# voithru/voice-activity-detection

Hardware: AMD Instinct MI355X
Metric: audio frames/sec (whole node) (higher is better)
Workload: dtype f32 (bf16x6 split operands, f32 accumulate)

## Files before the change

### voice_activity_detection_amd/csrc/savad.hip

```cpp
#include "savad_kernels.h"
#include "savad_kernels_bf16.h"
#include "savad_attn_pw_bf16.h"
#include "savad_packed_bf16.h"
#include "savad_kernels_f32s.h"
#include "savad_generic.h"
#include <type_traits>
#include "savad_logmel.h"
#include "savad_frontend.h"
#include "savad_ingest.h"
#include "savad_post.h"
#include "savad_post_device.h"
#include "savad_schedule.h"

#include <math.h>
#include <stdarg.h>
#include <stdio.h>
#include <string.h>

#include <functional>
#include <map>
#include <mutex>
#include <string>
#include <vector>

// ... 40 lines not shown
    size_t raw_floats = 0, packed_floats = 0;
    bool dirty = true;
    float* d_pe = nullptr;
    int pe_len = 0;
    std::vector<float> h_pe;
    int splits = 0;
    int row_mode = 0;
    bool batch_invariant = false;
    int precision = 0;
    char* d_frag3 = nullptr;
    size_t frag3_bytes = 0;
    bool frag3_dirty = true;
    bool lds_attrs3_set = false;
    size_t f3_win = 0;
    unsigned* d_sat = nullptr;
    char* d_frag = nullptr;
    size_t frag_bytes = 0;
    bool frag_dirty = true;
    bool lds_attrs_set = false;
    int n_cu = 256;
    size_t f_win = 0;
    struct LayerFrag {
        size_t wqkv, wo, w1, w2;
        size_t wqkv_vo = 0;
    };
    std::vector<LayerFrag> lf;
    std::vector<LayerFrag> lf3;
    int prof_capacity = 0, prof_used = 0, prof_nk = 0, prof_skip = 0;
    std::vector<hipEvent_t> events;
    std::vector<const char*> knames;

    size_t r_win, r_bin, r_lnf_w, r_lnf_b, r_wc, r_bc;
    struct LayerRaw {
        size_t wq, bq, wk, bk, wv, bv, wo, bo, ln1w, ln1b, w1, b1, w2, b2, ln2w, ln2b;
    };
    std::vector<LayerRaw> lr;
    struct LayerPacked {
        size_t wqkv, bqkv, w1, b1;
        size_t wvo, bqkv_vo;
        size_t frag;
    };
    std::vector<LayerPacked> lp;
    size_t p_wc, p_bc;
    size_t p_bias = 0;
    int FP = 0;
    size_t p_win_pad = 0;
};

namespace {

using namespace savad;

size_t add_param(savad_model* m, const std::string& key, size_t numel) {
    const size_t off = m->raw_floats;
    m->params.push_back(Param{key, numel, off, false});
    m->raw_floats += (numel + 3) & ~size_t(3);
    return off;
}

static_assert(sched::D == D && sched::TILE == TILE && sched::F32_MAX_LAYERS == PACKED_MAX_LAYERS, "savad_schedule.h: savad_kernels.h sizes");
static_assert(sched::BF_BLK_BYTES == bf::BLK_BYTES && sched::BF_HBLK_FLOATS == bf::HBLK_FLOATS && sched::BF_HRES_BYTES == sizeof(bf::hres_t) &&
                  sched::BF16_MAX_LAYERS == bf::PACKED_BF16_MAX_LAYERS && sched::PW_GRID == bf::PW_GRID, "savad_schedule.h: bf16 sizes");
// ... 129 lines not shown
    m->frag_dirty = false;
    return SAVAD_OK;
}

int pack_frags3(savad_model* m, hipStream_t st, const float* W, int N, int K, size_t off) {
    const size_t total = (size_t)N * K;
    const int grid = (int)((total + 255) / 256 < 1024 ? (total + 255) / 256 : 1024);
    hipLaunchKernelGGL(fs::pack_weight_frags3_kernel, dim3(grid), dim3(256), 0, st, W, N, K, reinterpret_cast<__bf16*>(m->d_frag3 + off));
    HIP_TRY(hipGetLastError());
    return SAVAD_OK;
}

int prepare_frags3(savad_model* m, hipStream_t st) {
    if (!m->frag3_dirty) return SAVAD_OK;
    const int L = m->cfg.num_layers;
    int rc;
    if ((rc = pack_frags3(m, st, win_fp32(m), D, m->FP, m->f3_win))) return rc;
    for (int l = 0; l < L; ++l) {
        if ((rc = pack_frags3(m, st, m->d_packed + m->lp[l].wqkv, 3 * D, D, m->lf3[l].wqkv))) return rc;
        if ((rc = pack_frags3(m, st, m->d_raw + m->lr[l].wo, D, D, m->lf3[l].wo))) return rc;
        if ((rc = pack_frags3(m, st, m->d_packed + m->lp[l].w1, DFF, D, m->lf3[l].w1))) return rc;
        if ((rc = pack_frags3(m, st, m->d_raw + m->lr[l].w2, D, DFF, m->lf3[l].w2))) return rc;
        const auto& p = m->lp[l];
        hipLaunchKernelGGL(fs::fold_vo_kernel, dim3(D), dim3(D), 0, st, m->d_raw + m->lr[l].wo, m->d_packed + p.wqkv + (size_t)2 * D * D,
                           m->d_packed + p.bqkv, m->d_packed + p.wvo, m->d_packed + p.bqkv_vo);
        HIP_TRY(hipGetLastError());
        if ((rc = pack_frags3(m, st, m->d_packed + p.wqkv, 2 * D, D, m->lf3[l].wqkv_vo))) return rc;
        if ((rc = pack_frags3(m, st, m->d_packed + p.wvo, D, D, m->lf3[l].wqkv_vo + (size_t)2 * D * D * 6))) return rc;
    }
    m->frag3_dirty = false;
    return SAVAD_OK;
}

template <typename KernelT>
int allow_lds(KernelT kernel, int bytes) {
    HIP_TRY(hipFuncSetAttribute(reinterpret_cast<const void*>(kernel), hipFuncAttributeMaxDynamicSharedMemorySize, bytes));
    return SAVAD_OK;
}

struct Prof {
    savad_model* m;
    hipStream_t st;
    hipEvent_t* ev;
    int n;
    Prof(savad_model* mm, hipStream_t s) : m(mm), st(s), ev(nullptr), n(0) {
        if (m->prof_capacity > 0 && m->prof_skip > 0) {
            --m->prof_skip;
        } else if (m->prof_capacity > 0 && m->prof_used < m->prof_capacity) {
            ev = m->events.data() + (size_t)m->prof_used * MAX_EVENTS;
            m->knames.clear();
            hipEventRecord(ev[0], st);
// ... 195 lines not shown
        r.wk = add_param(m, p + "self_attention.key_projection.weight", (size_t)D * D);
        r.bk = add_param(m, p + "self_attention.key_projection.bias", D);
        r.wv = add_param(m, p + "self_attention.value_projection.weight", (size_t)D * D);
        r.bv = add_param(m, p + "self_attention.value_projection.bias", D);
        r.wo = add_param(m, p + "self_attention.final_projection.weight", (size_t)D * D);
        r.bo = add_param(m, p + "self_attention.final_projection.bias", D);
        r.ln1w = add_param(m, p + "self_attention_sublayer.layer_norm.weight", D);
        r.ln1b = add_param(m, p + "self_attention_sublayer.layer_norm.bias", D);
        r.w1 = add_param(m, p + "feed_forward.feed_forward.0.weight", (size_t)DFF * D);
        r.b1 = add_param(m, p + "feed_forward.feed_forward.0.bias", DFF);
        r.w2 = add_param(m, p + "feed_forward.feed_forward.3.weight", (size_t)D * DFF);
        r.b2 = add_param(m, p + "feed_forward.feed_forward.3.bias", D);
        r.ln2w = add_param(m, p + "feed_forward_sublayer.layer_norm.weight", D);
        r.ln2b = add_param(m, p + "feed_forward_sublayer.layer_norm.bias", D);
        auto& q = m->lp[l];
        q.wqkv = m->packed_floats;
        m->packed_floats += (size_t)3 * D * D;
        q.bqkv = m->packed_floats;
        m->packed_floats += 3 * D;
        q.w1 = m->packed_floats;
        m->packed_floats += (size_t)DFF * D;
        q.b1 = m->packed_floats;
        m->packed_floats += DFF;
        q.wvo = m->packed_floats;
        m->packed_floats += (size_t)D * D;
        q.bqkv_vo = m->packed_floats;
        m->packed_floats += 3 * D;
        q.frag = m->packed_floats;
        m->packed_floats += FRAG_LAYER;
    }
    m->r_lnf_w = add_param(m, "encoder.layer_norm.weight", D);
    m->r_lnf_b = add_param(m, "encoder.layer_norm.bias", D);
    m->r_wc = add_param(m, "classifier.weight", 2 * D);
    m->r_bc = add_param(m, "classifier.bias", 2);
    m->p_bias = m->packed_floats;
    m->packed_floats += (size_t)L * LBIAS;
    m->p_wc = m->packed_floats;
    m->packed_floats += 2 * D;
    m->p_bc = m->packed_floats;
    m->packed_floats += 4;
    m->FP = (F + 15) / 16 * 16;
    m->p_win_pad = m->packed_floats;
    m->packed_floats += (size_t)D * m->FP;
    m->lf.resize(L);
    m->f_win = 0;
    m->frag_bytes = (size_t)D * ((F + 15) / 16 * 16) * 2;
    for (int l = 0; l < L; ++l) {
        auto& fl = m->lf[l];
        fl.wqkv = m->frag_bytes;
        m->frag_bytes += (size_t)3 * D * D * 2;
        fl.wo = m->frag_bytes;
        m->frag_bytes += (size_t)D * D * 2;
        fl.w1 = m->frag_bytes;
        m->frag_bytes += (size_t)DFF * D * 2;
        fl.w2 = m->frag_bytes;
        m->frag_bytes += (size_t)D * DFF * 2;
    }
    m->lf3.resize(L);
    m->f3_win = 0;
    m->frag3_bytes = (size_t)D * ((F + 15) / 16 * 16) * 6;
    for (int l = 0; l < L; ++l) {
        auto& fl = m->lf3[l];
        fl.wqkv = m->frag3_bytes;
        m->frag3_bytes += (size_t)3 * D * D * 6;
        fl.wo = m->frag3_bytes;
        m->frag3_bytes += (size_t)D * D * 6;
        fl.w1 = m->frag3_bytes;
        m->frag3_bytes += (size_t)DFF * D * 6;
        fl.w2 = m->frag3_bytes;
        m->frag3_bytes += (size_t)D * DFF * 6;
        fl.wqkv_vo = m->frag3_bytes;
        m->frag3_bytes += (size_t)3 * D * D * 6;
    }
    hipError_t e = hipMalloc(&m->d_raw, sizeof(float) * m->raw_floats);
    if (e == hipSuccess) e = hipMalloc(&m->d_frag, m->frag_bytes);
    if (e == hipSuccess) e = hipMalloc(&m->d_frag3, m->frag3_bytes);
    if (e == hipSuccess) e = hipMalloc(&m->d_sat, sizeof(unsigned));
    if (e == hipSuccess) e = hipMemset(m->d_sat, 0, sizeof(unsigned));
    if (e == hipSuccess) e = hipMalloc(&m->d_packed, sizeof(float) * m->packed_floats);
    if (e != hipSuccess) {
        if (m->d_raw) hipFree(m->d_raw);
        delete m;
        return fail(SAVAD_E_HIP, "hipMalloc(weights): %s", hipGetErrorString(e));
    }
    *out = m;
    return SAVAD_OK;
}

SAVAD_EXPORT void savad_destroy(savad_handle m) {
    if (!m) return;
    for (hipEvent_t e : m->events) hipEventDestroy(e);
    if (m->d_raw) hipFree(m->d_raw);
    if (m->d_packed) hipFree(m->d_packed);
    if (m->d_frag) hipFree(m->d_frag);
    if (m->d_frag3) hipFree(m->d_frag3);
// ... 287 lines not shown
            else
                hipLaunchKernelGGL((bf::attention_kernel_bf16<NW>), grid_groups, wg, ring, st, qf, kf, vtf, ctxf, B, T, bp.NG);
            prof.mark("attention_bf16");
            if (last)
                hipLaunchKernelGGL((bf::row_kernel_bf16<true, NW>), dim3(grid_rows), wg, ring + 9 * D * 4, st, ctxf, A);
            else
                hipLaunchKernelGGL((bf::row_kernel_bf16<false, NW>), dim3(grid_rows), wg, ring + 9 * D * 4, st, ctxf, A);
            prof.mark(last ? "row_last_bf16" : "row_bf16");
        }
    };
    if (bp.wide)
        run(std::integral_constant<int, 8>{});
    else
        run(std::integral_constant<int, 4>{});
    prof.done();
    HIP_TRY(hipGetLastError());
    return SAVAD_OK;
}


int prepare_f32s_launch(savad_model* m) {
    int rc;
    if (m->lds_attrs3_set) return SAVAD_OK;
    if ((rc = allow_lds(fs::input_qkv_kernel_f32s, fs::NRING3 * fs::SLOT_BYTES + 3 * D * 4))) return rc;
    if ((rc = allow_lds(fs::attention_row_kernel_f32s<false, false>, fs::ROW_LDS_BYTES))) return rc;
    if ((rc = allow_lds(fs::attention_row_kernel_f32s<true, false>, fs::ROW_LDS_BYTES))) return rc;
    if ((rc = allow_lds(fs::attention_row_kernel_f32s<false, true>, fs::ROW_LDS_BYTES))) return rc;
    if ((rc = allow_lds(fs::attention_row_kernel_f32s<true, true>, fs::ROW_LDS_BYTES))) return rc;
    if ((rc = allow_lds(fs::packed_forward_kernel_f32s, fs::packed_f32s_lds_bytes(fs::PACKED_F32S_MAX_LAYERS)))) return rc;
    if ((rc = allow_lds(fs::packed_forward_kernel_f32s_ns, fs::nsf_lds_bytes(fs::PACKED_F32S_MAX_LAYERS)))) return rc;
    m->lds_attrs3_set = true;
    return SAVAD_OK;
}

void launch_packed_forward_f32s(savad_model* m, int variant, hipStream_t st, const float* x, int B, int T, int F, float* out, const WindowOffsets& wo,
                                int win_base) {
    const int L = m->cfg.num_layers;
    const char* Fr = m->d_frag3;
    const int G = 32 / T, nblk = (B + G - 1) / G;
    fs::PackedF32sModel pm;
    for (int l = 0; l < fs::PACKED_F32S_MAX_LAYERS; ++l) {
        const auto& f = m->lf3[l < L ? l : 0];
        pm.layer[l] = fs::PackedF32sLayer{Fr + f.wqkv, Fr + f.wo, Fr + f.w1, Fr + f.w2};
    }
    pm.win = Fr + m->f3_win;
    pm.bin = m->d_raw + m->r_bin;
// ... 19 lines not shown
    if (bp.pad) {
        float* xp = (float*)(W + bp.xpad);
        pad_features(st, x, (size_t)B * T, F, m->FP, xp);
        x = xp;
        F = m->FP;
    }
    const long xbs = xbs_in > 0 ? xbs_in : (long)T * F;
    const float c = qscale();
    const float* R = m->d_raw;
    const float* P = m->d_packed;
    const char* Fr = m->d_frag3;
    Prof prof(m, st);
    if (bp.form == sched::SINGLE) {
        WindowOffsets none;
        none.w = 0;
        launch_packed_forward_f32s(m, bp.variant, st, x, B, T, F, out, none, 0);
        prof.mark("packed_forward_f32s");
        prof.done();
        HIP_TRY(hipGetLastError());
        return SAVAD_OK;
    }
    char* sets[2][3] = {{W + bp.q, W + bp.k, W + bp.v}, {W + bp.q2, W + bp.k2, W + bp.v2}};
    const bool packed = !bp.fold_v;
    auto wqkv3 = [&](int l) { return Fr + (packed ? m->lf3[l].wqkv : m->lf3[l].wqkv_vo); };
    auto bqkv3 = [&](int l) { return P + (packed ? m->lp[l].bqkv : m->lp[l].bqkv_vo); };
    hipLaunchKernelGGL(fs::input_qkv_kernel_f32s, dim3(bp.nblk_pad / 4), dim3(256), fs::NRING3 * fs::SLOT_BYTES + 3 * D * 4, st, x, xbs, B, T, F,
                       bp.nblk, Fr + m->f3_win, R + m->r_bin, m->d_pe, wqkv3(0), bqkv3(0), hb, sets[0][0], sets[0][1], sets[0][2], c);
    prof.mark("input_qkv_f32s");
    const int NG = bp.NG;
    const dim3 grid(packed ? bp.nblk_pad / 4 : 8 * (((long)B * NG + 7) / 8));
    for (int l = 0; l < L; ++l) {
        const auto& r = m->lr[l];
        const auto& p = m->lp[l];
        const auto& f = m->lf3[l];
        const bool last = l + 1 == L;
        char** cur = sets[l & 1];
        char** nxt = sets[(l + 1) & 1];
        fs::RowArgs3 A;
        A.B = B;
        A.T = T;
        A.nblk = bp.nblk;
        A.hbuf = hb;
        A.wo_frag = Fr + f.wo;
        A.bo = R + r.bo;
        A.w1_frag = Fr + f.w1;
        A.b1 = P + p.b1;
        A.w2_frag = Fr + f.w2;
        A.b2 = R + r.b2;
        A.wn_frag = last ? nullptr : wqkv3(l + 1);
// ... 1445 lines not shown
```

### voice_activity_detection_amd/csrc/savad_kernels_f32s.h

```cpp
#pragma once
#include "savad_kernels_bf16.h"
#include <type_traits>

namespace savad {
#ifdef SAVAD_TIMING
__device__ long long g_savad_wg[1024][4];
#endif
namespace fs {

using bf::bf16x8;
using bf::u32x4;
using bf::ldfrag;
using bf::stfrag;
using bf::FRAG_BYTES;
using bf::slot_row;
using bf::AttnState;
using bf::attn_state_init;
using bf::online_softmax_shifted;

constexpr int TFRAG_BYTES = 3 * FRAG_BYTES;
constexpr int BLK3_BYTES = 8 * TFRAG_BYTES;
constexpr int SLOT_BYTES = 2 * BLK3_BYTES;
constexpr int NRING3 = 3;
constexpr int HBLK_BYTES = 32 * D * 4;
// ... 140 lines not shown
    __device__ __forceinline__ void piece_raw(const DmaJob& j) const {
        asm volatile(
            "s_add_u32 m0, %2, %3\n\t"
            "s_nop 0\n\t"
            "global_load_lds_dwordx4 %0, %1 offset:%4"
            :
            : "v"(voff[I / 4]), "s"(j.src), "s"(j.ldsb), "n"((I / 4) * 4096), "n"((I % 4) * 1024)
            : "memory", "scc");
    }
    __device__ __forceinline__ void issue_all(const DmaJob& j) const {
        if (SAVAD_ABLATE & 1) return;
        piece_raw<0>(j); piece_raw<1>(j); piece_raw<2>(j); piece_raw<3>(j); piece_raw<4>(j); piece_raw<5>(j);
        piece_raw<6>(j); piece_raw<7>(j); piece_raw<8>(j); piece_raw<9>(j); piece_raw<10>(j); piece_raw<11>(j);
    }
    template <int NEWER>
    __device__ __forceinline__ void acquire() const {
        if (SAVAD_ABLATE & 2) return;
        __builtin_amdgcn_s_waitcnt(bf::Ring<4>::vmcnt_imm(NEWER * PER));
        asm volatile("" ::: "memory");
        __syncthreads();
    }
};

template <bool SWAP, bool DMA>
__device__ __forceinline__ void gemm_slot(f32x16& acc0, f32x16& acc1, const char* slot, const Tri (&xp)[8], const Ring3& ring,
                                          const DmaJob& job) {
    if (SAVAD_ABLATE & 8) {
#pragma unroll
        for (int ks = 0; ks < 8; ++ks) mfma6x2<SWAP>(acc0, acc1, xp[7 - ks], xp[ks ^ 1], xp[ks]);
        return;
    }
    const unsigned a = (unsigned)(size_t)slot + (unsigned)ring.lane * 16u;
    u32x4 f[2][6];
#define SAVAD_G_LD(ks, i) asm volatile("ds_read_b128 %0, %1 offset:%2" : "=v"(f[(ks) & 1][i]) : "v"(a), "n"(((i) / 3) * BLK3_BYTES + (ks) * TFRAG_BYTES + ((i) % 3) * FRAG_BYTES))
#define SAVAD_G_LD6(ks) SAVAD_G_LD(ks, 0); SAVAD_G_LD(ks, 1); SAVAD_G_LD(ks, 2); SAVAD_G_LD(ks, 3); SAVAD_G_LD(ks, 4); SAVAD_G_LD(ks, 5)
#define SAVAD_G_STEP(ks, P0, P1)                                                                                              \
    {                                                                                                                         \
        if constexpr ((ks) + 1 < 8) { SAVAD_G_LD6((ks) + 1); }                                                                \
        asm volatile("s_waitcnt lgkmcnt(%6)"                                                                                  \
                     : "+v"(f[(ks) & 1][0]), "+v"(f[(ks) & 1][1]), "+v"(f[(ks) & 1][2]), "+v"(f[(ks) & 1][3]), "+v"(f[(ks) & 1][4]), \
                       "+v"(f[(ks) & 1][5])                                                                                   \
                     : "n"((ks) + 1 < 8 ? 6 : 0));                                                                            \
        const Tri w0_{__builtin_bit_cast(bf16x8, f[(ks) & 1][0]), __builtin_bit_cast(bf16x8, f[(ks) & 1][1]),                  \
                      __builtin_bit_cast(bf16x8, f[(ks) & 1][2])};                                                            \
        const Tri w1_{__builtin_bit_cast(bf16x8, f[(ks) & 1][3]), __builtin_bit_cast(bf16x8, f[(ks) & 1][4]),                  \
                      __builtin_bit_cast(bf16x8, f[(ks) & 1][5])};                                                            \
        mfma6x2_lo<SWAP>(acc0, acc1, w0_, w1_, xp[ks]);                                                                       \
        if constexpr (DMA && (P1) >= 0) ring.template piece<((P1) >= 0 ? (P1) : 0)>(job);                                     \
        mfma6x2_hi<SWAP>(acc0, acc1, w0_, w1_, xp[ks]);                                                                       \
        if constexpr (DMA) ring.template piece<P0>(job);                                                                      \
    }
    SAVAD_G_LD6(0);
    SAVAD_G_STEP(0, 1, 0) SAVAD_G_STEP(1, 2, -1) SAVAD_G_STEP(2, 4, 3) SAVAD_G_STEP(3, 5, -1)
    SAVAD_G_STEP(4, 7, 6) SAVAD_G_STEP(5, 8, -1) SAVAD_G_STEP(6, 10, 9) SAVAD_G_STEP(7, 11, -1)
#undef SAVAD_G_STEP
#undef SAVAD_G_LD6
#undef SAVAD_G_LD
}

__global__ void pack_weight_frags3_kernel(const float* __restrict__ W, int N, int K, __bf16* __restrict__ out) {
    const int KS = K / 16;
    const size_t total = (size_t)(N / 32) * KS * 64 * 8;
    for (size_t i = (size_t)blockIdx.x * blockDim.x + threadIdx.x; i < total; i += (size_t)gridDim.x * blockDim.x) {
        const int e = (int)(i & 7);
        const int lane = (int)((i >> 3) & 63);
        const size_t f = i >> 9;
        const int ks = (int)(f % KS);
        const int nblk = (int)(f / KS);
        const int n = lane & 31, h = lane >> 5;
        const int k = 32 * (ks >> 1) + 16 * (ks & 1) + 8 * (e >> 2) + 4 * h + (e & 3);
        __bf16 ph, pm, pl;
        split1(W[(size_t)(32 * nblk + n) * K + k], ph, pm, pl);
        const size_t o = f * 3 * 512 + (size_t)lane * 8 + e;
        out[o] = ph;
        out[o + 512] = pm;
        out[o + 1024] = pl;
    }
}

__global__ void fold_vo_kernel(const float* __restrict__ Wo, const float* __restrict__ Wv, const float* __restrict__ bqkv,
                               float* __restrict__ Wvo, float* __restrict__ bqkv_vo) {
    const int n = blockIdx.x, k = threadIdx.x;
    double acc = 0.0, accb = 0.0;
    for (int j = 0; j < D; ++j) {
        const double w = (double)Wo[(size_t)n * D + j];
        acc += w * (double)Wv[(size_t)j * D + k];
        accb += w * (double)bqkv[2 * D + j];
    }
    Wvo[(size_t)n * D + k] = (float)acc;
    if (k == 0) bqkv_vo[2 * D + n] = (float)accb;
    if (n < 2) bqkv_vo[n * D + k] = bqkv[n * D + k];
}

template <int S, bool DMA>
__device__ __forceinline__ void qkv_slot(const char* slot, const Tri (&xp)[8], const float* lbq, char* __restrict__ qf, char* __restrict__ kf,
                                         char* __restrict__ vtf, int blk, const Ring3& ring, const DmaJob& job, float qscale, bool live) {
    const int lane = ring.lane, n = lane & 31, h = lane >> 5;
    constexpr int rb = S >> 1, nb0 = 2 * (S & 1);
    f32x16 acc[2];
    if constexpr (rb < 2) {
#pragma unroll
        for (int i = 0; i < 2; ++i) acc[i] = bias_block(lbq + D * rb + 32 * (nb0 + i), h);
        gemm_slot<false, DMA>(acc[0], acc[1], slot, xp, ring, job);
    } else {
#pragma unroll
        for (int i = 0; i < 2; ++i) {
            const float bv = lbq[2 * D + 32 * (nb0 + i) + n];
#pragma unroll
            for (int r = 0; r < 16; ++r) acc[i][r] = bv;
        }
        gemm_slot<true, DMA>(acc[0], acc[1], slot, xp, ring, job);
    }
    if constexpr (rb == 0) {
        acc[0] *= qscale;
        acc[1] *= qscale;
    }
    if (!live) return;
    char* dst = rb == 0 ? qf : (rb == 1 ? kf : vtf);
#pragma unroll
    for (int i = 0; i < 2; ++i)
#pragma unroll
        for (int j = 0; j < 2; ++j)
            sttri(dst + (size_t)blk * BLK3_BYTES + (2 * (nb0 + i) + j) * TFRAG_BYTES + lane * 16, split_half(acc[i], j));
}

__device__ __forceinline__ Tri load_x_tri(const float* p, bool valid) {
    f32x4 a = __builtin_nontemporal_load(reinterpret_cast<const f32x4*>(p)), b = __builtin_nontemporal_load(reinterpret_cast<const f32x4*>(p + 8));
    if (!valid) a = b = f32x4{0.f, 0.f, 0.f, 0.f};
    float t[8];
#pragma unroll
    for (int e = 0; e < 4; ++e) {
        t[e] = a[e];
        t[4 + e] = b[e];
    }
    return split8(t);
}

__device__ __forceinline__ void input_gemm_f32s(f32x16 (&h0)[4], const float* xr, bool valid, const char* win, int KS, int lane, int h) {
    constexpr int KSMAX = 8;
    f32x4 xa[KSMAX], xc[KSMAX];
#pragma unroll
    for (int ks = 0; ks < KSMAX; ++ks) {
        const int kc = ks < KS ? ks : KS - 1;
        const float* px = xr + 32 * (kc >> 1) + 16 * (kc & 1) + 4 * h;
        xa[ks] = __builtin_nontemporal_load(reinterpret_cast<const f32x4*>(px));
        xc[ks] = __builtin_nontemporal_load(reinterpret_cast<const f32x4*>(px + 8));
    }
// ... 7 lines not shown
#pragma unroll
                for (int nb = 0; nb < 4; ++nb) wn[nb] = wtri(nb, ks + 1);
            }
            float t[8];
#pragma unroll
            for (int e = 0; e < 4; ++e) {
                t[e] = valid ? xa[ks][e] : 0.0f;
                t[4 + e] = valid ? xc[ks][e] : 0.0f;
            }
            const Tri xf = split8(t);
            mfma6x2<false>(h0[0], h0[1], w0, w1, xf);
            mfma6x2<false>(h0[2], h0[3], w2, w3, xf);
        }
    for (int ks = KSMAX; ks < KS; ++ks) {
        const int f0 = 32 * (ks >> 1) + 16 * (ks & 1) + 4 * h;
        const Tri xf = load_x_tri(xr + f0, valid);
#pragma unroll
        for (int nb = 0; nb < 4; nb += 2)
            mfma6x2<false>(h0[nb], h0[nb + 1], ldtri(win + (size_t)(nb * KS + ks) * TFRAG_BYTES + lane * 16),
                           ldtri(win + (size_t)((nb + 1) * KS + ks) * TFRAG_BYTES + lane * 16), xf);
    }
}

__global__ __launch_bounds__(256, 1) void input_qkv_kernel_f32s(const float* __restrict__ x, long xbs, int B, int T, int F, int nblk,
                                                                const char* __restrict__ win_frag, const float* __restrict__ bin,
                                                                const float* __restrict__ pe, const char* __restrict__ wqkv_frag,
                                                                const float* __restrict__ bqkv, float* __restrict__ hbuf,
                                                                char* __restrict__ qf, char* __restrict__ kf, char* __restrict__ vtf,
                                                                float qscale) {
    extern __shared__ __attribute__((aligned(16))) char smem[];
    float* lbq = reinterpret_cast<float*>(smem + NRING3 * SLOT_BYTES);
    const int lane = threadIdx.x & 63, m = lane & 31, h = lane >> 5;
    const int w = __builtin_amdgcn_readfirstlane(threadIdx.x >> 6);
    const int blk = blockIdx.x * 4 + w;
    const Ring3 ring(smem, w, lane);
    auto job = [&](int t) { return ring.job(t, wqkv_frag + (size_t)(2 * t) * BLK3_BYTES, wqkv_frag + (size_t)(2 * t + 1) * BLK3_BYTES); };
    SAVAD_STAMP(57);
    ring.issue_all(job(0));
    ring.issue_all(job(1));
    stage_bias(lbq, bqkv, 3 * D);
    SAVAD_STAMP(58);
    size_t row;
    int t_frame;
    const bool valid = (blk < nblk) && slot_row(B, T, blk, m, row, t_frame);
    if (!valid) {
        row = 0;
        t_frame = 0;
    }
    f32x16 h0[4];
#pragma unroll
    for (int nb = 0; nb < 4; ++nb) {
        h0[nb] = zero16();
        add_bias(h0[nb], bin + 32 * nb, h);
        add_block(h0[nb], pe + (size_t)t_frame * D + 32 * nb, h);
    }
    input_gemm_f32s(h0, x + x_row_offset(row, T, F, xbs), valid, win_frag, F / 16, lane, h);
    SAVAD_STAMP(59);
    const bool live = blk < nblk;
    if (live) store_hblock32(hbuf + (size_t)blk * (32 * D), h0, lane);
    f32x4 xg[16];
    layernorm_regs(h0, xg);
    Tri xp[8];
    split_row(xg, xp);
    SAVAD_STAMP(60);
    const DmaJob none{nullptr, 0u};
#define SAVAD_IQ_STEP(T_)                                                                                                      \
    ring.acquire<((T_) + 1 < 6) ? 1 : 0>();                                                                                    \
    qkv_slot<T_, ((T_) + 2 < 6)>(ring.slot(T_), xp, lbq, qf, kf, vtf, blk, ring, (T_) + 2 < 6 ? job((T_) + 2) : none, qscale, live);
    SAVAD_IQ_STEP(0) SAVAD_IQ_STEP(1)
    SAVAD_STAMP(61);
    SAVAD_IQ_STEP(2) SAVAD_IQ_STEP(3)
    SAVAD_STAMP(62);
    SAVAD_IQ_STEP(4) SAVAD_IQ_STEP(5)
    SAVAD_STAMP(63);
#undef SAVAD_IQ_STEP
}

typedef __bf16 bf16x2 __attribute__((ext_vector_type(2)));
__device__ __forceinline__ void split_pair(float a0, float a1, unsigned& h, unsigned& m, unsigned& l) {
    __bf16 h0, m0, l0, h1, m1, l1;
    split1(a0, h0, m0, l0);
    split1(a1, h1, m1, l1);
    h = __builtin_bit_cast(unsigned, bf16x2{h0, h1});
    m = __builtin_bit_cast(unsigned, bf16x2{m0, m1});
    l = __builtin_bit_cast(unsigned, bf16x2{l0, l1});
}
__device__ __forceinline__ void settle_reference(f32x16& sc, AttnState& st, bool first ) {
    float mx = sc[0];
#pragma unroll
    for (int r = 1; r < 16; ++r) mx = fmaxf(mx, sc[r]);
    mx = half_max(mx);
    const bool move = (mx > RESCALE_LOG2) || (first && mx < -RESCALE_LOG2);
    if (__any(move)) {
        const float d = move ? mx : 0.0f;
        if (!first) {
            const float alpha = __builtin_amdgcn_exp2f(-d);
            st.l_run *= alpha;
#pragma unroll
// ... 138 lines not shown
    const float* b1;
    const char* w2_frag;
    const float* b2;
    const char* wn_frag;
    const float* wc;
    const float* bn;
    char *qf, *kf, *vtf;
    float* out;
    float qscale;
};
__device__ __forceinline__ const char* row_seg(const RowArgs3& A, int t, int sgm, bool folded) {
    if (!folded) {
        if (t < 2) return A.wo_frag + (size_t)(2 * t + sgm) * BLK3_BYTES;
        t -= 2;
    }
    if (t < 16) {
        const int c = t >> 2, r = t & 3;
        return r < 2 ? A.w1_frag + (size_t)(4 * c + 2 * r + sgm) * BLK3_BYTES
                     : A.w2_frag + (size_t)((2 * (r - 2) + sgm) * 32 + 8 * c) * TFRAG_BYTES;
    }
    return A.wn_frag + (size_t)(2 * (t - 16) + sgm) * BLK3_BYTES;
}

template <bool LAST>
struct RowBiases {
    BiasPiece pieces[4];
    BiasRegs<4> regs;
    float bc;
    float* lbn;
    __device__ __forceinline__ RowBiases(const RowArgs3& A, char* smem) {
        float* lbo = reinterpret_cast<float*>(smem + NRING3 * SLOT_BYTES);
        float* lb1 = lbo + D;
        float* lb2 = lb1 + DFF;
        lbn = lb2 + D;
        pieces[0] = BiasPiece{lbo, A.bo, D};
        pieces[1] = BiasPiece{lb1, A.b1, DFF};
        pieces[2] = BiasPiece{lb2, A.b2, D};
        pieces[3] = BiasPiece{lbn, LAST ? A.wc : A.bn, LAST ? 2 * D : 3 * D};
        regs = request_bias_pieces(pieces);
        bc = LAST ? A.bn[threadIdx.x & 1] : 0.0f;
    }
    __device__ __forceinline__ void commit() const {
        commit_bias_pieces(pieces, regs);
        if (LAST && threadIdx.x < 2) lbn[2 * D + threadIdx.x] = bc;
    }
};

template <bool LAST, bool FOLDED>
__device__ __forceinline__ void row_stage_f32s(const RowArgs3& A, char* smem, Tri (&xp)[8], const f32x16 (&hc)[4], f32x4 (&hr)[16], int blk,
                                               bool live, const Ring3& ring, int base) {
    float* lbo = reinterpret_cast<float*>(smem + NRING3 * SLOT_BYTES);
    float* lb1 = lbo + D;
    float* lb2 = lb1 + DFF;
    float* lbn = lb2 + D;
    const int lane = ring.lane, m = lane & 31, h = lane >> 5;
    constexpr int OFF = FOLDED ? 0 : 2;
    constexpr int NSLOT = OFF + (LAST ? 16 : 22);
    auto job = [&](int t) { return ring.job(base + t, row_seg(A, t, 0, FOLDED), row_seg(A, t, 1, FOLDED)); };
    const DmaJob none{nullptr, 0u};
#define SAVAD_ROW_GEMM(T_, acc0, acc1, operand)                                                                               \
    if ((T_) < 8) SAVAD_STAMP(24 + 3 * (T_));                                                                                 \
    if constexpr (!(FOLDED && (T_) == 0)) ring.acquire<((T_) + 1 < NSLOT) ? 1 : 0>();    \
    if ((T_) < 8) SAVAD_STAMP(25 + 3 * (T_));                                                                                 \
    gemm_slot<false, ((T_) + 2 < NSLOT)>(acc0, acc1, ring.slot(base + (T_)), operand, ring, (T_) + 2 < NSLOT ? job((T_) + 2) : none); \
    if ((T_) < 8) SAVAD_STAMP(26 + 3 * (T_));
    float* hb = A.hbuf + (size_t)blk * (32 * D);
    f32x16 h1[4];
    if constexpr (FOLDED) {
        ring.acquire<1>();
        landed_hblock32(hr);
#pragma unroll
        for (int nb = 0; nb < 4; ++nb) {
            h1[nb] = bias_block(lbo + 32 * nb, h) + hc[nb];
#pragma unroll
            for (int r = 0; r < 16; ++r) h1[nb][r] += hr[4 * nb + (r >> 2)][r & 3];
        }
    } else {
        ring.issue_all(job(0));
        ring.issue_all(job(1));
        ring.acquire<1>();
// ... 22 lines not shown
        _Pragma("unroll") for (int nbl = 0; nbl < 4; ++nbl) a[nbl] = bias_block(lb1 + 128 * (ch) + 32 * nbl, h);              \
        SAVAD_ROW_GEMM(OFF + 4 * (ch), a[0], a[1], xp)                                                                        \
        SAVAD_ROW_GEMM(OFF + 1 + 4 * (ch), a[2], a[3], xp)                                                                          \
        if ((ch) == 0) SAVAD_STAMP(20);                                                                                       \
        Tri ap[8];                                                                                                            \
        _Pragma("unroll") for (int nbl = 0; nbl < 4; ++nbl) {                                                                 \
            _Pragma("unroll") for (int r = 0; r < 16; ++r) a[nbl][r] = fmaxf(a[nbl][r], 0.0f);                                \
            ap[2 * nbl] = split_half(a[nbl], 0);                                                                              \
            ap[2 * nbl + 1] = split_half(a[nbl], 1);                                                                          \
        }                                                                                                                     \
        if ((ch) == 0) SAVAD_STAMP(21);                                                                                       \
        SAVAD_ROW_GEMM(OFF + 2 + 4 * (ch), o[0], o[1], ap)                                                                    \
        SAVAD_ROW_GEMM(OFF + 3 + 4 * (ch), o[2], o[3], ap)                                                                          \
        SAVAD_STAMP(7 + (ch));                                                                                                \
    }
    SAVAD_ROW_FFN(0) SAVAD_ROW_FFN(1) SAVAD_ROW_FFN(2) SAVAD_ROW_FFN(3)
#undef SAVAD_ROW_FFN
#undef SAVAD_ROW_GEMM
    if (!LAST && live) store_hblock32(hb, o, lane);
    layernorm_regs(o, xg);
    if constexpr (!LAST) {
        split_row(xg, xp);
        SAVAD_STAMP(11);
#define SAVAD_ROW_QKV(S_)                                                                                                     \
    ring.acquire<(OFF + 16 + (S_) + 1 < NSLOT) ? 1 : 0>();                                                                    \
    qkv_slot<S_, (OFF + 16 + (S_) + 2 < NSLOT)>(ring.slot(base + OFF + 16 + (S_)), xp, lbn, A.qf, A.kf, A.vtf, blk, ring,     \
                                                OFF + 16 + (S_) + 2 < NSLOT ? job(OFF + 16 + (S_) + 2) : none, A.qscale, live); \
    SAVAD_STAMP(12 + (S_));
        SAVAD_ROW_QKV(0) SAVAD_ROW_QKV(1) SAVAD_ROW_QKV(2) SAVAD_ROW_QKV(3) SAVAD_ROW_QKV(4) SAVAD_ROW_QKV(5)
#undef SAVAD_ROW_QKV
    } else {
        float z0 = 0.0f, z1 = 0.0f;
#pragma unroll
        for (int G = 0; G < 16; ++G) {
            const f32x4 c0 = ld4(lbn + 8 * G + 4 * h), c1 = ld4(lbn + D + 8 * G + 4 * h);
#pragma unroll
            for (int e = 0; e < 4; ++e) {
                z0 = __builtin_fmaf(xg[G][e], c0[e], z0);
                z1 = __builtin_fmaf(xg[G][e], c1[e], z1);
            }
        }
        z0 = half_sum(z0) + lbn[2 * D];
        z1 = half_sum(z1) + lbn[2 * D + 1];
        const float mx = fmaxf(z0, z1);
        const float lse = mx + logf(expf(z0 - mx) + expf(z1 - mx));
        size_t row;
        int t_frame;
        const bool valid = live && (blk < A.nblk) && slot_row(A.B, A.T, blk, m, row, t_frame);
        if (h == 0 && valid) *reinterpret_cast<f32x2*>(A.out + row * 2) = f32x2{z0 - lse, z1 - lse};
    }
}

template <bool LAST, bool PACKED>
__global__ __launch_bounds__(256, 1) void attention_row_kernel_f32s(const char* __restrict__ qf, const char* __restrict__ kf,
                                                                    const char* __restrict__ vtf, int NG, RowArgs3 A) {
    extern __shared__ __attribute__((aligned(16))) char smem[];
    const int B = A.B, T = A.T;
    const int lane = threadIdx.x & 63, m = lane & 31, h = lane >> 5;
    const int w = __builtin_amdgcn_readfirstlane(threadIdx.x >> 6);
    const Ring3 ring(smem, w, lane);
    AttnState st;
    attn_state_init(st);
    Tri qp[8];
    int blk_q, base = 0;
    bool active, qvalid;
    f32x4 hr[16];
#pragma unroll
    for (int i = 0; i < 16; ++i) hr[i] = f32x4{0.f, 0.f, 0.f, 0.f};
    SAVAD_STAMP(0);
#ifdef SAVAD_TIMING
    if (threadIdx.x == 0 && blockIdx.x < 1024) {
        g_savad_wg[blockIdx.x][0] = __builtin_readcyclecounter();
        g_savad_wg[blockIdx.x][2] = __builtin_amdgcn_s_memrealtime();
    }
#endif
    const RowBiases<LAST> biases(A, smem);
    if constexpr (PACKED) {
        biases.commit();
        blk_q = blockIdx.x * 4 + w;
        active = blk_q < A.nblk;
        const int G = 32 / T;
        qvalid = active && (m < G * T) && (blk_q * G + m / T < B);
        if (active) {
#pragma unroll
            for (int ks = 0; ks < 8; ++ks) qp[ks] = ldtri(qf + (size_t)blk_q * BLK3_BYTES + ks * TFRAG_BYTES + lane * 16);
            bool keyok[16];
#pragma unroll
            for (int r = 0; r < 16; ++r) {
                const int jk = 8 * (r >> 2) + 4 * h + (r & 3);
                keyok[r] = (jk < G * T) && (jk / T == m / T) && (blk_q * G + jk / T < B);
            }
            auto mask = [&](f32x16& sc) {
#pragma unroll
                for (int r = 0; r < 16; ++r) sc[r] = keyok[r] ? sc[r] : NEG_BIG;
            };
            attn_tile3_global(st, qp, kf + (size_t)blk_q * BLK3_BYTES, vtf + (size_t)blk_q * BLK3_BYTES, mask, lane);
        }
    } else {
        const int QB = (T + 31) / 32;
// ... 647 lines not shown
```

Before: 80.75 million.

## Fold Wq·Wkᵀ into query projection, store raw x as keys

Precomputes Wkᵀ·Wq (scaled by log2e/sqrt(D)) and its bias so the folded path emits a transformed query plus the V·O image, and writes the split input row directly as the key fragment instead of computing a K projection. This drops one of the three per-row QKV GEMM slots in both the input and row kernels (6→4 slots, 22→20 ring slots), and interleaves the K stores between MFMA halves through a new mid-callback hook. In exchange it adds a host-side fold kernel, changes the numerical path for attention scores, and drops the key bias term. That is valid only because a bias on K is constant across keys per query and cancels in softmax.

```diff
diff --git a/voice_activity_detection_amd/csrc/savad.hip b/voice_activity_detection_amd/csrc/savad.hip
--- a/voice_activity_detection_amd/csrc/savad.hip
+++ b/voice_activity_detection_amd/csrc/savad.hip
@@ -86,7 +86,7 @@
     size_t f_win = 0;
     struct LayerFrag {
         size_t wqkv, wo, w1, w2;
-        size_t wqkv_vo = 0;
+        size_t wq_vo = 0;
     };
     std::vector<LayerFrag> lf;
     std::vector<LayerFrag> lf3;
@@ -101,7 +101,7 @@
     std::vector<LayerRaw> lr;
     struct LayerPacked {
         size_t wqkv, bqkv, w1, b1;
-        size_t wvo, bqkv_vo;
+        size_t wq_vo, bq_vo;
         size_t frag;
     };
     std::vector<LayerPacked> lp;
@@ -277,11 +277,14 @@
         if ((rc = pack_frags3(m, st, m->d_packed + m->lp[l].w1, DFF, D, m->lf3[l].w1))) return rc;
         if ((rc = pack_frags3(m, st, m->d_raw + m->lr[l].w2, D, DFF, m->lf3[l].w2))) return rc;
         const auto& p = m->lp[l];
-        hipLaunchKernelGGL(fs::fold_vo_kernel, dim3(D), dim3(D), 0, st, m->d_raw + m->lr[l].wo, m->d_packed + p.wqkv + (size_t)2 * D * D,
-                           m->d_packed + p.bqkv, m->d_packed + p.wvo, m->d_packed + p.bqkv_vo);
+        const float* wqkv = m->d_packed + p.wqkv;
+        hipLaunchKernelGGL(fs::fold_qk_kernel, dim3(D), dim3(D), 0, st, wqkv, wqkv + (size_t)D * D, m->d_packed + p.bqkv,
+                           1.4426950408889634 / sqrt((double)D), m->d_packed + p.wq_vo, m->d_packed + p.bq_vo);
         HIP_TRY(hipGetLastError());
-        if ((rc = pack_frags3(m, st, m->d_packed + p.wqkv, 2 * D, D, m->lf3[l].wqkv_vo))) return rc;
-        if ((rc = pack_frags3(m, st, m->d_packed + p.wvo, D, D, m->lf3[l].wqkv_vo + (size_t)2 * D * D * 6))) return rc;
+        hipLaunchKernelGGL(fs::fold_vo_kernel, dim3(D), dim3(D), 0, st, m->d_raw + m->lr[l].wo, wqkv + (size_t)2 * D * D, m->d_packed + p.bqkv,
+                           m->d_packed + p.wq_vo + (size_t)D * D, m->d_packed + p.bq_vo + D);
+        HIP_TRY(hipGetLastError());
+        if ((rc = pack_frags3(m, st, m->d_packed + p.wq_vo, 2 * D, D, m->lf3[l].wq_vo))) return rc;
     }
     m->frag3_dirty = false;
     return SAVAD_OK;
@@ -523,10 +526,10 @@
         m->packed_floats += (size_t)DFF * D;
         q.b1 = m->packed_floats;
         m->packed_floats += DFF;
-        q.wvo = m->packed_floats;
-        m->packed_floats += (size_t)D * D;
-        q.bqkv_vo = m->packed_floats;
-        m->packed_floats += 3 * D;
+        q.wq_vo = m->packed_floats;
+        m->packed_floats += (size_t)2 * D * D;
+        q.bq_vo = m->packed_floats;
+        m->packed_floats += 2 * D;
         q.frag = m->packed_floats;
         m->packed_floats += FRAG_LAYER;
     }
@@ -570,8 +573,8 @@
         m->frag3_bytes += (size_t)DFF * D * 6;
         fl.w2 = m->frag3_bytes;
         m->frag3_bytes += (size_t)D * DFF * 6;
-        fl.wqkv_vo = m->frag3_bytes;
-        m->frag3_bytes += (size_t)3 * D * D * 6;
+        fl.wq_vo = m->frag3_bytes;
+        m->frag3_bytes += (size_t)2 * D * D * 6;
     }
     hipError_t e = hipMalloc(&m->d_raw, sizeof(float) * m->raw_floats);
     if (e == hipSuccess) e = hipMalloc(&m->d_frag, m->frag_bytes);
@@ -905,6 +908,7 @@
 int prepare_f32s_launch(savad_model* m) {
     int rc;
     if (m->lds_attrs3_set) return SAVAD_OK;
+    if ((rc = allow_lds(fs::input_qkv_kernel_f32s_plain, fs::NRING3 * fs::SLOT_BYTES + 3 * D * 4))) return rc;
     if ((rc = allow_lds(fs::input_qkv_kernel_f32s, fs::NRING3 * fs::SLOT_BYTES + 3 * D * 4))) return rc;
     if ((rc = allow_lds(fs::attention_row_kernel_f32s<false, false>, fs::ROW_LDS_BYTES))) return rc;
     if ((rc = allow_lds(fs::attention_row_kernel_f32s<true, false>, fs::ROW_LDS_BYTES))) return rc;
@@ -970,9 +974,10 @@
     }
     char* sets[2][3] = {{W + bp.q, W + bp.k, W + bp.v}, {W + bp.q2, W + bp.k2, W + bp.v2}};
     const bool packed = !bp.fold_v;
-    auto wqkv3 = [&](int l) { return Fr + (packed ? m->lf3[l].wqkv : m->lf3[l].wqkv_vo); };
-    auto bqkv3 = [&](int l) { return P + (packed ? m->lp[l].bqkv : m->lp[l].bqkv_vo); };
-    hipLaunchKernelGGL(fs::input_qkv_kernel_f32s, dim3(bp.nblk_pad / 4), dim3(256), fs::NRING3 * fs::SLOT_BYTES + 3 * D * 4, st, x, xbs, B, T, F,
+    auto wqkv3 = [&](int l) { return Fr + (packed ? m->lf3[l].wqkv : m->lf3[l].wq_vo); };
+    auto bqkv3 = [&](int l) { return P + (packed ? m->lp[l].bqkv : m->lp[l].bq_vo); };
+    const auto input_qkv = packed ? fs::input_qkv_kernel_f32s_plain : fs::input_qkv_kernel_f32s;
+    hipLaunchKernelGGL(input_qkv, dim3(bp.nblk_pad / 4), dim3(256), fs::NRING3 * fs::SLOT_BYTES + 3 * D * 4, st, x, xbs, B, T, F,
                        bp.nblk, Fr + m->f3_win, R + m->r_bin, m->d_pe, wqkv3(0), bqkv3(0), hb, sets[0][0], sets[0][1], sets[0][2], c);
     prof.mark("input_qkv_f32s");
     const int NG = bp.NG;
diff --git a/voice_activity_detection_amd/csrc/savad_kernels_f32s.h b/voice_activity_detection_amd/csrc/savad_kernels_f32s.h
--- a/voice_activity_detection_amd/csrc/savad_kernels_f32s.h
+++ b/voice_activity_detection_amd/csrc/savad_kernels_f32s.h
@@ -186,9 +186,13 @@
     }
 };
 
-template <bool SWAP, bool DMA>
+struct NoMid {
+    template <int KS>
+    __device__ __forceinline__ void operator()(std::integral_constant<int, KS>) const {}
+};
+template <bool SWAP, bool DMA, class Mid = NoMid>
 __device__ __forceinline__ void gemm_slot(f32x16& acc0, f32x16& acc1, const char* slot, const Tri (&xp)[8], const Ring3& ring,
-                                          const DmaJob& job) {
+                                          const DmaJob& job, const Mid& mid = Mid{}) {
     if (SAVAD_ABLATE & 8) {
 #pragma unroll
         for (int ks = 0; ks < 8; ++ks) mfma6x2<SWAP>(acc0, acc1, xp[7 - ks], xp[ks ^ 1], xp[ks]);
@@ -211,6 +215,7 @@
                       __builtin_bit_cast(bf16x8, f[(ks) & 1][5])};                                                            \
         mfma6x2_lo<SWAP>(acc0, acc1, w0_, w1_, xp[ks]);                                                                       \
         if constexpr (DMA && (P1) >= 0) ring.template piece<((P1) >= 0 ? (P1) : 0)>(job);                                     \
+        mid(std::integral_constant<int, (ks)>{});                                                                             \
         mfma6x2_hi<SWAP>(acc0, acc1, w0_, w1_, xp[ks]);                                                                       \
         if constexpr (DMA) ring.template piece<P0>(job);                                                                      \
     }
@@ -243,7 +248,7 @@
 }
 
 __global__ void fold_vo_kernel(const float* __restrict__ Wo, const float* __restrict__ Wv, const float* __restrict__ bqkv,
-                               float* __restrict__ Wvo, float* __restrict__ bqkv_vo) {
+                               float* __restrict__ Wvo, float* __restrict__ bvo) {
     const int n = blockIdx.x, k = threadIdx.x;
     double acc = 0.0, accb = 0.0;
     for (int j = 0; j < D; ++j) {
@@ -252,41 +257,93 @@
         accb += w * (double)bqkv[2 * D + j];
     }
     Wvo[(size_t)n * D + k] = (float)acc;
-    if (k == 0) bqkv_vo[2 * D + n] = (float)accb;
-    if (n < 2) bqkv_vo[n * D + k] = bqkv[n * D + k];
-}
-
-template <int S, bool DMA>
-__device__ __forceinline__ void qkv_slot(const char* slot, const Tri (&xp)[8], const float* lbq, char* __restrict__ qf, char* __restrict__ kf,
-                                         char* __restrict__ vtf, int blk, const Ring3& ring, const DmaJob& job, float qscale, bool live) {
+    if (k == 0) bvo[n] = (float)accb;
+}
+
+__global__ void fold_qk_kernel(const float* __restrict__ Wq, const float* __restrict__ Wk, const float* __restrict__ bq, double c,
+                               float* __restrict__ Wqt, float* __restrict__ bqt) {
+    const int n = blockIdx.x, k = threadIdx.x;
+    double acc = 0.0, accb = 0.0;
+    for (int o = 0; o < D; ++o) {
+        const double w = (double)Wk[(size_t)o * D + n];
+        acc += w * (double)Wq[(size_t)o * D + k];
+        accb += w * (double)bq[o];
+    }
+    Wqt[(size_t)n * D + k] = (float)(c * acc);
+    if (k == 0) bqt[n] = (float)(c * accb);
+}
+
+template <int RB, int HALF, bool DMA, bool SCALE, class Mid = NoMid>
+__device__ __forceinline__ void qkv_slot(const char* slot, const Tri (&xp)[8], const float* lb, char* __restrict__ dst, int blk,
+                                         const Ring3& ring, const DmaJob& job, float qscale, bool live, const Mid& mid = Mid{}) {
     const int lane = ring.lane, n = lane & 31, h = lane >> 5;
-    constexpr int rb = S >> 1, nb0 = 2 * (S & 1);
+    constexpr int nb0 = 2 * HALF;
     f32x16 acc[2];
-    if constexpr (rb < 2) {
-#pragma unroll
-        for (int i = 0; i < 2; ++i) acc[i] = bias_block(lbq + D * rb + 32 * (nb0 + i), h);
-        gemm_slot<false, DMA>(acc[0], acc[1], slot, xp, ring, job);
+    if constexpr (RB < 2) {
+#pragma unroll
+        for (int i = 0; i < 2; ++i) acc[i] = bias_block(lb + 32 * (nb0 + i), h);
+        gemm_slot<false, DMA>(acc[0], acc[1], slot, xp, ring, job, mid);
     } else {
 #pragma unroll
         for (int i = 0; i < 2; ++i) {
-            const float bv = lbq[2 * D + 32 * (nb0 + i) + n];
+            const float bv = lb[32 * (nb0 + i) + n];
 #pragma unroll
             for (int r = 0; r < 16; ++r) acc[i][r] = bv;
         }
-        gemm_slot<true, DMA>(acc[0], acc[1], slot, xp, ring, job);
-    }
-    if constexpr (rb == 0) {
+        gemm_slot<true, DMA>(acc[0], acc[1], slot, xp, ring, job, mid);
+    }
+    if constexpr (SCALE) {
         acc[0] *= qscale;
         acc[1] *= qscale;
     }
     if (!live) return;
-    char* dst = rb == 0 ? qf : (rb == 1 ? kf : vtf);
 #pragma unroll
     for (int i = 0; i < 2; ++i)
 #pragma unroll
         for (int j = 0; j < 2; ++j)
             sttri(dst + (size_t)blk * BLK3_BYTES + (2 * (nb0 + i) + j) * TFRAG_BYTES + lane * 16, split_half(acc[i], j));
 }
+template <int S, bool QKF, bool DMA, class Mid = NoMid>
+__device__ __forceinline__ void qkv_image_slot(const char* slot, const Tri (&xp)[8], const float* lbq, char* __restrict__ qf, char* __restrict__ kf,
+                                               char* __restrict__ vtf, int blk, const Ring3& ring, const DmaJob& job, float qscale, bool live,
+                                               const Mid& mid = Mid{}) {
+    constexpr int pos = S >> 1, rb = QKF ? 2 * pos : pos;
+    qkv_slot<rb, (S & 1), DMA, (rb == 0 && !QKF)>(slot, xp, lbq + D * pos, rb == 0 ? qf : (rb == 1 ? kf : vtf), blk, ring, job, qscale, live, mid);
+}
+
+#ifndef SAVAD_KSTORE
+#define SAVAD_KSTORE 2
+#endif
+__device__ __forceinline__ void store_k_tri(char* kblk , const Tri (&xp)[8], int ks, int lane) {
+    sttri(kblk + ks * TFRAG_BYTES + lane * 16, xp[ks]);
+}
+__device__ __forceinline__ void store_k_burst(char* kblk, const Tri (&xp)[8], int lane, bool live) {
+    if (!live) return;
+#pragma unroll
+    for (int ks = 0; ks < 8; ++ks) store_k_tri(kblk, xp, ks, lane);
+}
+template <int S>
+struct KStoreMid {
+    char* kblk;
+    const Tri (&xp)[8];
+    int lane;
+    bool live;
+    template <int KS>
+    __device__ __forceinline__ void operator()(std::integral_constant<int, KS>) const {
+        if constexpr ((KS & 1) && ((SAVAD_KSTORE == 2 && S == 0) || SAVAD_KSTORE == 3)) {
+            __builtin_amdgcn_sched_barrier(SAVAD_PIECE_FENCE);
+            if (live) {
+                if constexpr (SAVAD_KSTORE == 2) {
+                    store_k_tri(kblk, xp, KS - 1, lane);
+                    store_k_tri(kblk, xp, KS, lane);
+                } else {
+                    store_k_tri(kblk, xp, 4 * S + (KS >> 1), lane);
+                }
+            }
+            __builtin_amdgcn_sched_barrier(SAVAD_PIECE_FENCE);
+        }
+    }
+};
 
 __device__ __forceinline__ Tri load_x_tri(const float* p, bool valid) {
     f32x4 a = __builtin_nontemporal_load(reinterpret_cast<const f32x4*>(p)), b = __builtin_nontemporal_load(reinterpret_cast<const f32x4*>(p + 8));
@@ -340,13 +397,11 @@
     }
 }
 
-__global__ __launch_bounds__(256, 1) void input_qkv_kernel_f32s(const float* __restrict__ x, long xbs, int B, int T, int F, int nblk,
-                                                                const char* __restrict__ win_frag, const float* __restrict__ bin,
-                                                                const float* __restrict__ pe, const char* __restrict__ wqkv_frag,
-                                                                const float* __restrict__ bqkv, float* __restrict__ hbuf,
-                                                                char* __restrict__ qf, char* __restrict__ kf, char* __restrict__ vtf,
-                                                                float qscale) {
-    extern __shared__ __attribute__((aligned(16))) char smem[];
+template <bool QKF>
+__device__ __forceinline__ void input_qkv_f32s(char* smem, const float* __restrict__ x, long xbs, int B, int T, int F, int nblk,
+                                               const char* __restrict__ win_frag, const float* __restrict__ bin, const float* __restrict__ pe,
+                                               const char* __restrict__ wqkv_frag, const float* __restrict__ bqkv, float* __restrict__ hbuf,
+                                               char* __restrict__ qf, char* __restrict__ kf, char* __restrict__ vtf, float qscale) {
     float* lbq = reinterpret_cast<float*>(smem + NRING3 * SLOT_BYTES);
     const int lane = threadIdx.x & 63, m = lane & 31, h = lane >> 5;
     const int w = __builtin_amdgcn_readfirstlane(threadIdx.x >> 6);
@@ -356,7 +411,7 @@
     SAVAD_STAMP(57);
     ring.issue_all(job(0));
     ring.issue_all(job(1));
-    stage_bias(lbq, bqkv, 3 * D);
+    stage_bias(lbq, bqkv, (QKF ? 2 : 3) * D);
     SAVAD_STAMP(58);
     size_t row;
     int t_frame;
@@ -382,16 +437,46 @@
     split_row(xg, xp);
     SAVAD_STAMP(60);
     const DmaJob none{nullptr, 0u};
-#define SAVAD_IQ_STEP(T_)                                                                                                      \
-    ring.acquire<((T_) + 1 < 6) ? 1 : 0>();                                                                                    \
-    qkv_slot<T_, ((T_) + 2 < 6)>(ring.slot(T_), xp, lbq, qf, kf, vtf, blk, ring, (T_) + 2 < 6 ? job((T_) + 2) : none, qscale, live);
-    SAVAD_IQ_STEP(0) SAVAD_IQ_STEP(1)
-    SAVAD_STAMP(61);
-    SAVAD_IQ_STEP(2) SAVAD_IQ_STEP(3)
-    SAVAD_STAMP(62);
-    SAVAD_IQ_STEP(4) SAVAD_IQ_STEP(5)
-    SAVAD_STAMP(63);
+    constexpr int NS = QKF ? 4 : 6;
+    char* kblk = kf + (size_t)blk * BLK3_BYTES;
+#define SAVAD_IQ_STEP(T_, mid)                                                                                                 \
+    ring.acquire<((T_) + 1 < NS) ? 1 : 0>();                                                                                   \
+    if (QKF && SAVAD_KSTORE == 1 && (T_) == 0) store_k_burst(kblk, xp, lane, live);                                            \
+    qkv_image_slot<T_, QKF, ((T_) + 2 < NS)>(ring.slot(T_), xp, lbq, qf, kf, vtf, blk, ring, (T_) + 2 < NS ? job((T_) + 2) : none, qscale, \
+                                             live, mid);
+    if constexpr (QKF) {
+        if (SAVAD_KSTORE == 0) store_k_burst(kblk, xp, lane, live);
+        SAVAD_IQ_STEP(0, (KStoreMid<0>{kblk, xp, lane, live})) SAVAD_IQ_STEP(1, (KStoreMid<1>{kblk, xp, lane, live}))
+        SAVAD_STAMP(61);
+        SAVAD_IQ_STEP(2, NoMid{}) SAVAD_IQ_STEP(3, NoMid{})
+        SAVAD_STAMP(63);
+    } else {
+        SAVAD_IQ_STEP(0, NoMid{}) SAVAD_IQ_STEP(1, NoMid{})
+        SAVAD_STAMP(61);
+        SAVAD_IQ_STEP(2, NoMid{}) SAVAD_IQ_STEP(3, NoMid{})
+        SAVAD_STAMP(62);
+        SAVAD_IQ_STEP(4, NoMid{}) SAVAD_IQ_STEP(5, NoMid{})
+        SAVAD_STAMP(63);
+    }
 #undef SAVAD_IQ_STEP
+}
+__global__ __launch_bounds__(256, 1) void input_qkv_kernel_f32s(const float* __restrict__ x, long xbs, int B, int T, int F, int nblk,
+                                                                const char* __restrict__ win_frag, const float* __restrict__ bin,
+                                                                const float* __restrict__ pe, const char* __restrict__ wqkv_frag,
+                                                                const float* __restrict__ bqkv, float* __restrict__ hbuf,
+                                                                char* __restrict__ qf, char* __restrict__ kf, char* __restrict__ vtf,
+                                                                float qscale) {
+    extern __shared__ __attribute__((aligned(16))) char smem[];
+    input_qkv_f32s<true>(smem, x, xbs, B, T, F, nblk, win_frag, bin, pe, wqkv_frag, bqkv, hbuf, qf, kf, vtf, qscale);
+}
+__global__ __launch_bounds__(256, 1) void input_qkv_kernel_f32s_plain(const float* __restrict__ x, long xbs, int B, int T, int F, int nblk,
+                                                                      const char* __restrict__ win_frag, const float* __restrict__ bin,
+                                                                      const float* __restrict__ pe, const char* __restrict__ wqkv_frag,
+                                                                      const float* __restrict__ bqkv, float* __restrict__ hbuf,
+                                                                      char* __restrict__ qf, char* __restrict__ kf, char* __restrict__ vtf,
+                                                                      float qscale) {
+    extern __shared__ __attribute__((aligned(16))) char smem[];
+    input_qkv_f32s<false>(smem, x, xbs, B, T, F, nblk, win_frag, bin, pe, wqkv_frag, bqkv, hbuf, qf, kf, vtf, qscale);
 }
 
 typedef __bf16 bf16x2 __attribute__((ext_vector_type(2)));
@@ -576,7 +661,7 @@
     return A.wn_frag + (size_t)(2 * (t - 16) + sgm) * BLK3_BYTES;
 }
 
-template <bool LAST>
+template <bool LAST, bool FOLDED>
 struct RowBiases {
     BiasPiece pieces[4];
     BiasRegs<4> regs;
@@ -590,7 +675,7 @@
         pieces[0] = BiasPiece{lbo, A.bo, D};
         pieces[1] = BiasPiece{lb1, A.b1, DFF};
         pieces[2] = BiasPiece{lb2, A.b2, D};
-        pieces[3] = BiasPiece{lbn, LAST ? A.wc : A.bn, LAST ? 2 * D : 3 * D};
+        pieces[3] = BiasPiece{lbn, LAST ? A.wc : A.bn, (LAST || FOLDED) ? 2 * D : 3 * D};
         regs = request_bias_pieces(pieces);
         bc = LAST ? A.bn[threadIdx.x & 1] : 0.0f;
     }
@@ -609,7 +694,7 @@
     float* lbn = lb2 + D;
     const int lane = ring.lane, m = lane & 31, h = lane >> 5;
     constexpr int OFF = FOLDED ? 0 : 2;
-    constexpr int NSLOT = OFF + (LAST ? 16 : 22);
+    constexpr int NSLOT = OFF + (LAST ? 16 : FOLDED ? 20 : 22);
     auto job = [&](int t) { return ring.job(base + t, row_seg(A, t, 0, FOLDED), row_seg(A, t, 1, FOLDED)); };
     const DmaJob none{nullptr, 0u};
 #define SAVAD_ROW_GEMM(T_, acc0, acc1, operand)                                                                               \
@@ -678,12 +763,21 @@
     if constexpr (!LAST) {
         split_row(xg, xp);
         SAVAD_STAMP(11);
-#define SAVAD_ROW_QKV(S_)                                                                                                     \
+        char* kblk = A.kf + (size_t)blk * BLK3_BYTES;
+#define SAVAD_ROW_QKV(S_, mid)                                                                                                \
     ring.acquire<(OFF + 16 + (S_) + 1 < NSLOT) ? 1 : 0>();                                                                    \
-    qkv_slot<S_, (OFF + 16 + (S_) + 2 < NSLOT)>(ring.slot(base + OFF + 16 + (S_)), xp, lbn, A.qf, A.kf, A.vtf, blk, ring,     \
-                                                OFF + 16 + (S_) + 2 < NSLOT ? job(OFF + 16 + (S_) + 2) : none, A.qscale, live); \
+    if (FOLDED && SAVAD_KSTORE == 1 && (S_) == 0) store_k_burst(kblk, xp, lane, live);                                        \
+    qkv_image_slot<S_, FOLDED, (OFF + 16 + (S_) + 2 < NSLOT)>(ring.slot(base + OFF + 16 + (S_)), xp, lbn, A.qf, A.kf, A.vtf, blk, ring, \
+                                                              OFF + 16 + (S_) + 2 < NSLOT ? job(OFF + 16 + (S_) + 2) : none, A.qscale, live, mid); \
     SAVAD_STAMP(12 + (S_));
-        SAVAD_ROW_QKV(0) SAVAD_ROW_QKV(1) SAVAD_ROW_QKV(2) SAVAD_ROW_QKV(3) SAVAD_ROW_QKV(4) SAVAD_ROW_QKV(5)
+        if constexpr (FOLDED) {
+            if (SAVAD_KSTORE == 0) store_k_burst(kblk, xp, lane, live);
+            SAVAD_ROW_QKV(0, (KStoreMid<0>{kblk, xp, lane, live})) SAVAD_ROW_QKV(1, (KStoreMid<1>{kblk, xp, lane, live}))
+            SAVAD_ROW_QKV(2, NoMid{}) SAVAD_ROW_QKV(3, NoMid{})
+        } else {
+            SAVAD_ROW_QKV(0, NoMid{}) SAVAD_ROW_QKV(1, NoMid{}) SAVAD_ROW_QKV(2, NoMid{}) SAVAD_ROW_QKV(3, NoMid{}) SAVAD_ROW_QKV(4, NoMid{})
+            SAVAD_ROW_QKV(5, NoMid{})
+        }
 #undef SAVAD_ROW_QKV
     } else {
         float z0 = 0.0f, z1 = 0.0f;
@@ -730,7 +824,7 @@
         g_savad_wg[blockIdx.x][2] = __builtin_amdgcn_s_memrealtime();
     }
 #endif
-    const RowBiases<LAST> biases(A, smem);
+    const RowBiases<LAST, !PACKED> biases(A, smem);
     if constexpr (PACKED) {
         biases.commit();
         blk_q = blockIdx.x * 4 + w;
```

After: 84.42 million, median of 6. +4.5%, better.
